# LPD-EPFL/AggregaThor

Measured on NVIDIA H100. Metric: steps/sec (whole box, device-timed, max over ranks) ResNet-50 slim + Krum f=2, higher is better.
Workload: dtype bf16

## Files before the change

### aggregathor_b200/native/op_nn/layers.cu

```cuda

#include <cuda_bf16.h>

#include <agb_device.cuh>

using namespace agb;

namespace {

using bf16 = __nv_bfloat16;

template<typename T> struct Oct;
template<> struct alignas(16) Oct<bf16> { uint4 raw; };
template<> struct alignas(16) Oct<float> { float4 lo, hi; };

__device__ __forceinline__ void unpack8(uint4 const& raw, float (&v)[8]) {
    __nv_bfloat162 const* h = reinterpret_cast<__nv_bfloat162 const*>(&raw);
#pragma unroll
    for (int i = 0; i < 4; ++i) {
        float2 f = __bfloat1622float2(h[i]);
        v[2 * i] = f.x;
        v[2 * i + 1] = f.y;
    }
}
__device__ __forceinline__ uint4 pack8(float const (&v)[8]) {
    uint4 raw;
    __nv_bfloat162* h = reinterpret_cast<__nv_bfloat162*>(&raw);
#pragma unroll
    for (int i = 0; i < 4; ++i)
        h[i] = __floats2bfloat162_rn(v[2 * i], v[2 * i + 1]);
    return raw;
}
__device__ __forceinline__ void unpack8(Oct<bf16> const& o, float (&v)[8]) { unpack8(o.raw, v); }
__device__ __forceinline__ void unpack8(Oct<float> const& o, float (&v)[8]) {
    v[0] = o.lo.x; v[1] = o.lo.y; v[2] = o.lo.z; v[3] = o.lo.w; v[4] = o.hi.x; v[5] = o.hi.y; v[6] = o.hi.z; v[7] = o.hi.w;
}
template<typename T> __device__ __forceinline__ Oct<T> pack_oct(float const (&v)[8]);
template<> __device__ __forceinline__ Oct<bf16> pack_oct<bf16>(float const (&v)[8]) { return Oct<bf16>{pack8(v)}; }
template<> __device__ __forceinline__ Oct<float> pack_oct<float>(float const (&v)[8]) {
    return Oct<float>{make_float4(v[0], v[1], v[2], v[3]), make_float4(v[4], v[5], v[6], v[7])};
}
template<typename T> __device__ __forceinline__ Oct<T> zero_oct() {
    float const z[8] = {0.f, 0.f, 0.f, 0.f, 0.f, 0.f, 0.f, 0.f};
    return pack_oct<T>(z);
}
template<typename T> __device__ __forceinline__ Oct<T> load_oct(T const* p) { return *reinterpret_cast<Oct<T> const*>(p); }
template<typename T> __device__ __forceinline__ void store_oct(T* p, Oct<T> const& o) { *reinterpret_cast<Oct<T>*>(p) = o; }
__device__ __forceinline__ float to_f(bf16 v) { return __bfloat162float(v); }
__device__ __forceinline__ float to_f(float v) { return v; }
template<typename T> __device__ __forceinline__ T from_f(float v);
template<> __device__ __forceinline__ bf16 from_f<bf16>(float v) { return __float2bfloat16(v); }
template<> __device__ __forceinline__ float from_f<float>(float v) { return v; }

constexpr int kThreads = 256;

// ... 786 lines not shown
            for (int kw = 0; kw < KW; ++kw) {
                int const tw = w + pad_l - kw;
                if (tw < 0 || tw % s)
                    continue;
                int const ow = tw / s;
                if (ow >= OW)
                    continue;
                float v[8];
                unpack8(load_oct(dcol + ((static_cast<long long>(n) * OH + oh) * OW + ow) * ldcol + (kh * KW + kw) * C + o * 8), v);
#pragma unroll
                for (int j = 0; j < 8; ++j)
                    acc[j] += v[j];
            }
        }
        store_oct(dx + i * 8, pack_oct<T>(acc));
    }
}

inline int grid_for(long long work, int threads = kThreads, int cap = agb::sm_count() * 8) {
    long long blocks = (work + threads - 1) / threads;
    if (blocks > cap)
        blocks = cap;
    return blocks < 1 ? 1 : static_cast<int>(blocks);
}

struct SumsPlan {
    int rows_per_cta, strip;
    dim3 grid;
};
inline SumsPlan plan_sums(long long rows_per_group, int C, int groups) {
    int const octets = C >> 3;
    SumsPlan plan;
    plan.strip = 8;
    int const row_lanes = kThreads / plan.strip;
    int const strips = (octets + plan.strip - 1) / plan.strip;
    long long target = (agb::sm_count() * 6 + strips * groups - 1) / (strips * groups);
    if (target < 1)
        target = 1;
    long long rows_per_cta = (rows_per_group + target - 1) / target;
    long long const min_rows = static_cast<long long>(row_lanes) * kRowUnroll;
    if (rows_per_cta < min_rows)
        rows_per_cta = min_rows;
    plan.rows_per_cta = static_cast<int>(rows_per_cta);
    plan.grid = dim3(static_cast<unsigned>((rows_per_group + rows_per_cta - 1) / rows_per_cta), strips, groups);
    return plan;
}


constexpr int kFusedThreads = 512;
constexpr int kFusedScratchBytes = kFusedThreads * 16 * 4;
constexpr int kFusedPivotBytes = 12 * 1024;
constexpr int kFusedStashBytes = 180 * 1024;
using FusedSum = double;
constexpr long long kFusedHalfBytes = 16 + 2ll * 8 * 16384;

struct BnFused {
    bf16 const* a;
    bf16 const* b;
    bf16 const* mask;
    bf16* out;
    bf16* out2;
    float const* gamma;
    float const* beta;
    float* moving_mean;
    float* moving_var;
    float* save_mean;
    float* save_rstd;
    float* dgamma;
    float* dbeta;
    long long group_stride;
    unsigned* state;
    unsigned char* ws;
    long long rows_per_group, rows_per_cta;
    int C, groups, ctas_per_group, stash_vecs, relu, replicas;
    float eps, decay;
};

__device__ __forceinline__ unsigned ld_acquire_gpu(unsigned const* addr) {
    unsigned value;
    asm volatile("ld.acquire.gpu.global.u32 %0, [%1];" : "=r"(value) : "l"(addr) : "memory");
    return value;
}

template<bool BWD>
__global__ void __launch_bounds__(kFusedThreads, 1) bn_fused_kernel(BnFused const p) {
    pdl_trigger();
    pdl_wait();
    extern __shared__ __align__(16) unsigned char fused_smem[];
    float* red = reinterpret_cast<float*>(fused_smem);
    float* pivot_s = reinterpret_cast<float*>(fused_smem + kFusedScratchBytes);
    uint4* stash_a = reinterpret_cast<uint4*>(fused_smem + kFusedScratchBytes + kFusedPivotBytes);
    uint4* stash_b = stash_a + p.stash_vecs;
    int const octets = p.C >> 3;
    __shared__ unsigned slot_shared;
    float* chan = red;
    int const group = blockIdx.x / p.ctas_per_group, chunk = blockIdx.x % p.ctas_per_group;
    if (threadIdx.x == 0)
        slot_shared = __ldcg(p.state) & 1u;
    for (int c0 = threadIdx.x; c0 < p.C; c0 += 4 * kFusedThreads) {
        float first[4], second[4];
#pragma unroll
        for (int u = 0; u < 4; ++u) {
            int const c = c0 + u * kFusedThreads;
            first[u] = second[u] = 0.f;
            if (c < p.C) {
                first[u] = BWD ? p.save_mean[group * p.C + c] : (p.moving_mean ? p.moving_mean[c] : 0.f);
                second[u] = BWD ? p.save_rstd[group * p.C + c] : 0.f;
            }
        }
#pragma unroll
        for (int u = 0; u < 4; ++u) {
            int const c = c0 + u * kFusedThreads;
            if (c < p.C) {
                chan[c] = first[u];
                chan[p.C + c] = second[u];
                if (!BWD)
                    pivot_s[c] = first[u];
            }
        }
    }
    __syncthreads();
    unsigned const slot = slot_shared;
    unsigned char* mine = p.ws + slot * kFusedHalfBytes;
    unsigned* bar = reinterpret_cast<unsigned*>(mine);
    FusedSum* sums = reinterpret_cast<FusedSum*>(mine + 16);
    {
        uint4* other = reinterpret_cast<uint4*>(p.ws + (slot ^ 1u) * kFusedHalfBytes);
        for (long long i = static_cast<long long>(blockIdx.x) * kFusedThreads + threadIdx.x; i < kFusedHalfBytes / 16; i += static_cast<long long>(gridDim.x) * kFusedThreads)
            other[i] = make_uint4(0, 0, 0, 0);
    }
    long long const row_begin = static_cast<long long>(chunk) * p.rows_per_cta;
    long long const row_end = min(p.rows_per_group, row_begin + p.rows_per_cta);
    long long const nvec = row_end > row_begin ? (row_end - row_begin) * octets : 0;
    long long const base = (static_cast<long long>(group) * p.rows_per_group + row_begin) * octets;
    uint4 const* ga = reinterpret_cast<uint4 const*>(p.a) + base;
    uint4 const* gb = p.b ? reinterpret_cast<uint4 const*>(p.b) + base : nullptr;
    uint4* gout2 = (BWD && p.out2) ? reinterpret_cast<uint4*>(p.out2) + base : nullptr;
    uint4 const* gm = (BWD && p.mask) ? reinterpret_cast<uint4 const*>(p.mask) + base : nullptr;
    uint4* gout = reinterpret_cast<uint4*>(p.out) + base;
    int const stride = kFusedThreads - kFusedThreads % octets;
    int const lanes = stride / octets;
    bool const active = static_cast<int>(threadIdx.x) < stride;
    int const o = threadIdx.x % octets, lane = threadIdx.x / octets;
    int const cbase = group * p.C + o * 8;
    float s0[8], s1[8], mu[8], rs[8];
#pragma unroll
    for (int j = 0; j < 8; ++j) {
        s0[j] = 0.f;
        s1[j] = 0.f;
        mu[j] = active ? chan[o * 8 + j] : 0.f;
        rs[j] = active ? chan[p.C + o * 8 + j] : 0.f;
    }
    __syncthreads();
    if (active) {
        constexpr int U = BWD ? 4 : 8;
        for (long long i0 = threadIdx.x; i0 < nvec; i0 += static_cast<long long>(stride) * U) {
            uint4 ra[U], rb[U], rm[U];
#pragma unroll
            for (int u = 0; u < U; ++u) {
                long long const i = i0 + static_cast<long long>(u) * stride;
                if (i < nvec) {
                    ra[u] = ga[i];
                    if (BWD)
                        rb[u] = gb[i];
                    if (BWD && gm)
                        rm[u] = gm[i];
                    if (!BWD && gb && (i & 7) == 0)
                        asm volatile("prefetch.global.L2 [%0];" :: "l"(gb + i));
                }
            }
#pragma unroll
            for (int u = 0; u < U; ++u) {
                long long const i = i0 + static_cast<long long>(u) * stride;
                if (i >= nvec)
                    continue;
                float va[8];
                unpack8(ra[u], va);
                if (!BWD) {
#pragma unroll
                    for (int j = 0; j < 8; ++j) {
                        float const d = va[j] - mu[j];
                        s0[j] += d;
                        s1[j] += d * d;
                    }
                    if (i < p.stash_vecs)
                        stash_a[i] = ra[u];
                } else {
                    if (gm) {
                        float vy[8];
                        unpack8(rm[u], vy);
#pragma unroll
                        for (int j = 0; j < 8; ++j)
                            va[j] = vy[j] > 0.f ? va[j] : 0.f;
                        if (gout2)
                            gout2[i] = pack8(va);
                    }
                    float vx[8];
                    unpack8(rb[u], vx);
#pragma unroll
                    for (int j = 0; j < 8; ++j) {
                        s0[j] += va[j];
                        s1[j] += va[j] * (vx[j] - mu[j]) * rs[j];
                    }
                    if (i < p.stash_vecs) {
                        stash_a[i] = gm ? pack8(va) : ra[u];
                        stash_b[i] = rb[u];
                    }
                }
            }
        }
#pragma unroll
        for (int j = 0; j < 8; ++j) {
            red[lane * (octets * 16) + o * 16 + j] = s0[j];
            red[lane * (octets * 16) + o * 16 + 8 + j] = s1[j];
        }
    }
    __syncthreads();
    if (nvec > 0) {
        for (int t = threadIdx.x; t < octets * 16; t += kFusedThreads) {
            float total = 0.f;
            for (int l = 0; l < lanes; ++l)
                total += red[l * (octets * 16) + t];
            long long const slot_index = (static_cast<long long>(chunk % p.replicas) * p.groups + group) * p.C + (t >> 4) * 8 + (t & 7);
            atomicAdd(sums + slot_index * 2 + ((t >> 3) & 1), static_cast<FusedSum>(total));
        }
    }
    __threadfence();
    __syncthreads();
    if (threadIdx.x == 0) {
        atomicAdd(bar, 1u);
        unsigned spins = 0;
        while (ld_acquire_gpu(bar) < gridDim.x) {
            __nanosleep(200);
            if (++spins > (1u << 22)) {
                printf("[agb] bn_fused_kernel: grid barrier timeout (block %d, %u of %u arrived)\n", static_cast<int>(blockIdx.x), ld_acquire_gpu(bar), gridDim.x);
                __trap();
            }
        }
    }
    __syncthreads();
    if (blockIdx.x == 0 && threadIdx.x == 0)
        *p.state = slot ^ 1u;
    {
        double const n = static_cast<double>(p.rows_per_group), inv_n = 1.0 / n;
        for (int c = threadIdx.x; c < p.C; c += kFusedThreads) {
            long long const idx = static_cast<long long>(group) * p.C + c;
            double2 part[8];
#pragma unroll
            for (int r = 0; r < 8; ++r) {
                part[r] = make_double2(0., 0.);
                if (r < p.replicas)
                    part[r] = __ldcg(reinterpret_cast<double2 const*>(sums + (static_cast<long long>(r) * p.groups * p.C + idx) * 2));
            }
            float const gmc = p.gamma ? p.gamma[c] : 1.f;
            float const aux0 = BWD ? p.save_rstd[idx] : p.beta[c], aux1 = BWD ? p.save_mean[idx] : 0.f;
            double t0 = 0., t1 = 0.;
#pragma unroll
            for (int r = 0; r < 8; ++r) {
                t0 += part[r].x;
                t1 += part[r].y;
            }
            if (!BWD) {
                float const pivot = pivot_s[c];
                double const shifted = t0 * inv_n;
                double const mean = shifted + static_cast<double>(pivot);
                double var = fma(-shifted, shifted, t1 * inv_n);
                if (var < 0.)
                    var = 0.;
                float const rstd = rsqrtf(static_cast<float>(var) + p.eps);
                chan[c] = gmc * rstd;
                chan[p.C + c] = aux0 - static_cast<float>(mean) * gmc * rstd;
                if (chunk == 0) {
                    p.save_mean[idx] = static_cast<float>(mean);
                    p.save_rstd[idx] = rstd;
                    if (p.moving_mean && group == 0) {
                        double const unbiased = n > 1. ? var * n / (n - 1.) : var;
                        p.moving_mean[c] = p.decay * pivot + (1.f - p.decay) * static_cast<float>(mean);
                        p.moving_var[c] = p.decay * p.moving_var[c] + (1.f - p.decay) * static_cast<float>(unbiased);
                    }
                }
            } else {
                float const inv = static_cast<float>(inv_n), rsc = aux0, muc = aux1;
                float const b1 = -gmc * rsc * rsc * static_cast<float>(t1) * inv;
                chan[c] = gmc * rsc;
                chan[p.C + c] = b1;
                chan[2 * p.C + c] = -gmc * rsc * static_cast<float>(t0) * inv - b1 * muc;
                if (chunk == 0) {
                    if (p.dgamma)
                        p.dgamma[group * p.group_stride + c] = static_cast<float>(t1);
                    p.dbeta[group * p.group_stride + c] = static_cast<float>(t0);
                }
            }
        }
    }
    __syncthreads();
    if (!active)
        return;
    float c0[8], c1[8], c2[8];
#pragma unroll
    for (int j = 0; j < 8; ++j) {
        c0[j] = chan[o * 8 + j];
        c1[j] = chan[p.C + o * 8 + j];
        c2[j] = BWD ? chan[2 * p.C + o * 8 + j] : 0.f;
    }
    auto finish = [&](float (&va)[8], float const (&vx)[8]) {
        if (!BWD) {
#pragma unroll
            for (int j = 0; j < 8; ++j) {
                va[j] = va[j] * c0[j] + c1[j] + vx[j];
                if (p.relu)
                    va[j] = fmaxf(va[j], 0.f);
            }
        } else {
#pragma unroll
            for (int j = 0; j < 8; ++j)
                va[j] = c0[j] * va[j] + c1[j] * vx[j] + c2[j];
        }
        return pack8(va);
    };
    long long const resident_end = nvec < p.stash_vecs ? nvec : static_cast<long long>(p.stash_vecs);
    long long i = threadIdx.x;
    if (!BWD && gb) {
        constexpr int R = 4;
        for (; i < resident_end; i += static_cast<long long>(stride) * R) {
            uint4 rb[R];
#pragma unroll
            for (int u = 0; u < R; ++u) {
                long long const k = i + static_cast<long long>(u) * stride;
                if (k < resident_end)
                    rb[u] = gb[k];
            }
#pragma unroll
            for (int u = 0; u < R; ++u) {
                long long const k = i + static_cast<long long>(u) * stride;
                if (k >= resident_end)
                    continue;
                float va[8], vx[8];
                unpack8(stash_a[k], va);
                unpack8(rb[u], vx);
                gout[k] = finish(va, vx);
            }
        }
        i = static_cast<long long>(threadIdx.x) >= resident_end ? threadIdx.x : threadIdx.x + ((resident_end - 1 - threadIdx.x) / stride + 1) * stride;
    } else {
        for (; i < resident_end; i += stride) {
            float va[8], vx[8] = {0.f, 0.f, 0.f, 0.f, 0.f, 0.f, 0.f, 0.f};
            unpack8(stash_a[i], va);
            if (BWD)
                unpack8(stash_b[i], vx);
            gout[i] = finish(va, vx);
        }
    }
    constexpr int V = BWD ? 2 : 4;
    for (; i < nvec; i += static_cast<long long>(stride) * V) {
        uint4 ra[V], rb[V], rm[V];
#pragma unroll
        for (int u = 0; u < V; ++u) {
            long long const k = i + static_cast<long long>(u) * stride;
            if (k < nvec) {
                ra[u] = ga[k];
                if (gb)
                    rb[u] = gb[k];
                if (BWD && gm)
                    rm[u] = gm[k];
            }
        }
#pragma unroll
        for (int u = 0; u < V; ++u) {
            long long const k = i + static_cast<long long>(u) * stride;
            if (k >= nvec)
                continue;
            float va[8], vx[8] = {0.f, 0.f, 0.f, 0.f, 0.f, 0.f, 0.f, 0.f};
            unpack8(ra[u], va);
            if (gb)
                unpack8(rb[u], vx);
            if (BWD && gm) {
                float vy[8];
                unpack8(rm[u], vy);
#pragma unroll
                for (int j = 0; j < 8; ++j)
                    va[j] = vy[j] > 0.f ? va[j] : 0.f;
            }
            gout[k] = finish(va, vx);
        }
    }
}

long long g_fused_max_mb[2] = {72, 40};
long long g_fused_min_rows = 4096;

template<bool BWD>
int launch_bn_fused(BnFused p, long long rows, cudaStream_t s) {
    int const octets = p.C >> 3;
    if ((p.C & 7) || 3 * p.C * 4 > kFusedScratchBytes || p.C * 4 > kFusedPivotBytes || p.groups < 1 || p.groups > agb::sm_count() || rows % p.groups || static_cast<long long>(p.C) * p.groups > 16384)
        return 399;
    static bool configured = false;
    int const smem = kFusedScratchBytes + kFusedPivotBytes + kFusedStashBytes;
    if (!configured) {
        AGB_CUDA_OK(cudaFuncSetAttribute(bn_fused_kernel<BWD>, cudaFuncAttributeMaxDynamicSharedMemorySize, smem));
        configured = true;
    }
    bool const extra = BWD ? p.out2 != nullptr : p.b != nullptr;
    long long const bytes = rows * p.C * 2;
    if (rows < (extra ? g_fused_min_rows / 4 : g_fused_min_rows) || bytes > g_fused_max_mb[BWD ? 1 : 0] << 20)
        return 399;
    p.rows_per_group = rows / p.groups;
    long long const vecs = p.rows_per_group * octets;
    long long const min_vecs = octets * 32ll > 2048 ? octets * 32ll : 2048;
    long long want = (vecs + min_vecs - 1) / min_vecs;
    int const cap = agb::sm_count() / p.groups;
    p.ctas_per_group = static_cast<int>(want < 1 ? 1 : (want > cap ? cap : want));
    p.rows_per_cta = (p.rows_per_group + p.ctas_per_group - 1) / p.ctas_per_group;
    p.stash_vecs = kFusedStashBytes / 16 / (BWD ? 2 : 1);
    long long const room = 16384 / (static_cast<long long>(p.C) * p.groups);
    p.replicas = static_cast<int>(room < 1 ? 1 : (room > 8 ? 8 : room));
    if (p.replicas > p.ctas_per_group)
        p.replicas = p.ctas_per_group;
    AGB_CUDA_OK(launch_pdl(bn_fused_kernel<BWD>, dim3(p.groups * p.ctas_per_group), dim3(kFusedThreads), static_cast<size_t>(smem), s, p));
    AGB_CUDA_OK(cudaGetLastError());
    return 0;
}

template<int MODE, typename T>
int launch_sums(SumsPlan const& plan, cudaStream_t s, T const* a, T const* b, T const* y, float const* mean, float const* rstd, double* out,
                 long long rows_per_group, int C, SumsFinalize const& fin) {
    if (plan.strip == 32)
        AGB_CUDA_OK(launch_pdl(channel_sums_kernel<T, MODE, 32>, dim3(plan.grid), dim3(kThreads), 0, s, a, b, y, mean, rstd, out, rows_per_group, C, plan.rows_per_cta, fin));
    else if (plan.strip == 16)
        AGB_CUDA_OK(launch_pdl(channel_sums_kernel<T, MODE, 16>, dim3(plan.grid), dim3(kThreads), 0, s, a, b, y, mean, rstd, out, rows_per_group, C, plan.rows_per_cta, fin));
    else
        AGB_CUDA_OK(launch_pdl(channel_sums_kernel<T, MODE, 8>, dim3(plan.grid), dim3(kThreads), 0, s, a, b, y, mean, rstd, out, rows_per_group, C, plan.rows_per_cta, fin));
    return 0;
}

template<typename T>
int bn_forward_impl(void const* x, void const* residual, void* y, void const* gamma, void const* beta, void* moving_mean, void* moving_var, void* save_mean, void* save_rstd,
                   void* sums, void* scale, void* shift, long long rows, int C, int groups, float eps, float decay, int relu, void* stream) {
    if ((C & 7) || groups < 1 || rows % groups)
        return 301;
    cudaStream_t s = static_cast<cudaStream_t>(stream);
    long long const rpg = rows / groups;
    SumsFinalize fin{};
    fin.ticket = reinterpret_cast<unsigned*>(static_cast<double*>(sums) + 2 * C * groups);
    fin.gamma = static_cast<float const*>(gamma); fin.beta = static_cast<float const*>(beta);
    fin.save_mean = static_cast<float*>(save_mean); fin.save_rstd = static_cast<float*>(save_rstd);
    fin.scale = static_cast<float*>(scale); fin.shift = static_cast<float*>(shift);
    fin.moving_mean = static_cast<float*>(moving_mean); fin.moving_var = static_cast<float*>(moving_var);
    fin.groups = groups; fin.eps = eps; fin.decay = decay;
    SumsPlan plan = plan_sums(rpg, C, groups);
    if (int status = launch_sums<0, T>(plan, s, static_cast<T const*>(x), nullptr, nullptr, nullptr, nullptr, static_cast<double*>(sums), rpg, C, fin))
        return status;
    long long const octets = rows * (C >> 3);
    AGB_CUDA_OK(launch_pdl(bn_apply_kernel<T>, dim3(grid_for(octets)), dim3(kThreads), 0, s, static_cast<T const*>(x), static_cast<T const*>(residual), static_cast<T*>(y), static_cast<float const*>(scale), static_cast<float const*>(shift), octets, C, rpg, relu));
    AGB_CUDA_OK(cudaGetLastError());
    return 0;
}

template<typename T>
int bn_backward_impl(void const* dy, void const* x, void const* y, void const* gamma, void const* save_mean, void const* save_rstd, void* dx, void* dmasked, void* dgamma, void* dbeta,
                    void* sums, void* coef, long long rows, int C, int groups, long long group_stride, void* stream) {
    if ((C & 7) || groups < 1 || rows % groups)
        return 301;
    cudaStream_t s = static_cast<cudaStream_t>(stream);
    long long const rpg = rows / groups;
    SumsFinalize fin{};
    fin.ticket = reinterpret_cast<unsigned*>(static_cast<double*>(sums) + 2 * C * groups);
    fin.gamma = static_cast<float const*>(gamma);
    fin.save_mean = const_cast<float*>(static_cast<float const*>(save_mean)); fin.save_rstd = const_cast<float*>(static_cast<float const*>(save_rstd));
    fin.scale = static_cast<float*>(coef);
    fin.dgamma = static_cast<float*>(dgamma); fin.dbeta = static_cast<float*>(dbeta);
    fin.groups = groups; fin.group_stride = group_stride;
// ... 155 lines not shown
    size_t const stem_smem = static_cast<size_t>(kh) * W * C * sizeof(T);
    if ((C & 7) != 0 && stem_smem <= 40 * 1024 && static_cast<long long>(N) * OH < (1ll << 31)) {
        AGB_CUDA_OK(launch_pdl(im2col_stem_kernel<T>, dim3(static_cast<unsigned>(N * OH)), dim3(kThreads), stem_smem, static_cast<cudaStream_t>(stream), static_cast<T const*>(x), static_cast<T*>(col), H, W, C, OH, OW, kh, kw, s, pad_t, pad_l, ldcol));
        AGB_CUDA_OK(cudaGetLastError());
        return 0;
    }
    long long const work = (C & 7) == 0 ? static_cast<long long>(N) * OH * OW * kh * kw * (C >> 3) : static_cast<long long>(N) * OH * OW * (ldcol >> 3);
    AGB_CUDA_OK(launch_pdl(im2col_kernel<T>, dim3(grid_for(work, kThreads, agb::sm_count() * 16)), dim3(kThreads), 0, static_cast<cudaStream_t>(stream), static_cast<T const*>(x), static_cast<T*>(col), N, H, W, C, OH, OW, kh, kw, s, pad_t, pad_l, ldcol));
    AGB_CUDA_OK(cudaGetLastError());
    return 0;
}

template<typename T>
int col2im_impl(void const* dcol, void* dx, int N, int H, int W, int C, int OH, int OW, int kh, int kw, int s, int pad_t, int pad_l, long long ldcol, void* stream) {
    if ((C & 7) || (ldcol & 7))
        return 301;
    long long const work = static_cast<long long>(N) * H * W * (C >> 3);
    AGB_CUDA_OK(launch_pdl(col2im_kernel<T>, dim3(grid_for(work, kThreads, agb::sm_count() * 16)), dim3(kThreads), 0, static_cast<cudaStream_t>(stream), static_cast<T const*>(dcol), static_cast<T*>(dx), N, H, W, C, OH, OW, kh, kw, s, pad_t, pad_l, ldcol));
    AGB_CUDA_OK(cudaGetLastError());
    return 0;
}

}

extern "C" {

int agb_bn_forward(void const* x, void const* residual, void* y, void const* gamma, void const* beta, void* moving_mean, void* moving_var, void* save_mean, void* save_rstd,
                   void* sums, void* scale, void* shift, long long rows, int C, int groups, float eps, float decay, int relu, void* stream) {
    return bn_forward_impl<bf16>(x, residual, y, gamma, beta, moving_mean, moving_var, save_mean, save_rstd, sums, scale, shift, rows, C, groups, eps, decay, relu, stream);
}
int agb_bn_forward_f32(void const* x, void const* residual, void* y, void const* gamma, void const* beta, void* moving_mean, void* moving_var, void* save_mean, void* save_rstd,
                   void* sums, void* scale, void* shift, long long rows, int C, int groups, float eps, float decay, int relu, void* stream) {
    return bn_forward_impl<float>(x, residual, y, gamma, beta, moving_mean, moving_var, save_mean, save_rstd, sums, scale, shift, rows, C, groups, eps, decay, relu, stream);
}


int agb_bn_backward(void const* dy, void const* x, void const* y, void const* gamma, void const* save_mean, void const* save_rstd, void* dx, void* dmasked, void* dgamma, void* dbeta,
                    void* sums, void* coef, long long rows, int C, int groups, long long group_stride, void* stream) {
    return bn_backward_impl<bf16>(dy, x, y, gamma, save_mean, save_rstd, dx, dmasked, dgamma, dbeta, sums, coef, rows, C, groups, group_stride, stream);
}
int agb_bn_backward_f32(void const* dy, void const* x, void const* y, void const* gamma, void const* save_mean, void const* save_rstd, void* dx, void* dmasked, void* dgamma, void* dbeta,
                    void* sums, void* coef, long long rows, int C, int groups, long long group_stride, void* stream) {
    return bn_backward_impl<float>(dy, x, y, gamma, save_mean, save_rstd, dx, dmasked, dgamma, dbeta, sums, coef, rows, C, groups, group_stride, stream);
}


int agb_bn_fused_set_limits(long long forward_mb, long long backward_mb, long long min_rows) {
    g_fused_max_mb[0] = forward_mb;
    g_fused_max_mb[1] = backward_mb;
    g_fused_min_rows = min_rows;
    return 0;
}

long long agb_bn_fused_workspace_bytes() {
    return 16 + 2 * kFusedHalfBytes;
}

int agb_bn_forward_fused(void const* x, void const* residual, void* y, void const* gamma, void const* beta, void* moving_mean, void* moving_var, void* save_mean, void* save_rstd,
                         void* ws, long long rows, int C, int groups, float eps, float decay, int relu, void* stream) {
    BnFused p{};
    p.a = static_cast<bf16 const*>(x); p.b = static_cast<bf16 const*>(residual); p.out = static_cast<bf16*>(y);
    p.gamma = static_cast<float const*>(gamma); p.beta = static_cast<float const*>(beta);
    p.moving_mean = static_cast<float*>(moving_mean); p.moving_var = static_cast<float*>(moving_var);
    p.save_mean = static_cast<float*>(save_mean); p.save_rstd = static_cast<float*>(save_rstd);
    p.state = static_cast<unsigned*>(ws); p.ws = static_cast<unsigned char*>(ws) + 16;
    p.C = C; p.groups = groups; p.eps = eps; p.decay = decay; p.relu = relu;
    return launch_bn_fused<false>(p, rows, static_cast<cudaStream_t>(stream));
}

int agb_bn_backward_fused(void const* dy, void const* x, void const* y, void const* gamma, void const* save_mean, void const* save_rstd, void* dx, void* dmasked, void* dgamma,
                          void* dbeta, void* ws, long long rows, int C, int groups, long long group_stride, void* stream) {
    BnFused p{};
    p.a = static_cast<bf16 const*>(dy); p.b = static_cast<bf16 const*>(x); p.mask = static_cast<bf16 const*>(y); p.out = static_cast<bf16*>(dx);
    p.out2 = static_cast<bf16*>(dmasked);
    if (p.out2 && !p.mask)
        return 302;
    p.gamma = static_cast<float const*>(gamma);
    p.save_mean = const_cast<float*>(static_cast<float const*>(save_mean)); p.save_rstd = const_cast<float*>(static_cast<float const*>(save_rstd));
    p.dgamma = static_cast<float*>(dgamma); p.dbeta = static_cast<float*>(dbeta); p.group_stride = group_stride;
    p.state = static_cast<unsigned*>(ws); p.ws = static_cast<unsigned char*>(ws) + 16;
    p.C = C; p.groups = groups;
    return launch_bn_fused<true>(p, rows, static_cast<cudaStream_t>(stream));
}

int agb_colsum(void const* dy, void const* y, void* out, void* sums, long long rows, int C, int groups, long long group_stride, void* stream) {
    return colsum_impl<bf16>(dy, y, out, sums, rows, C, groups, group_stride, stream);
}
int agb_colsum_f32(void const* dy, void const* y, void* out, void* sums, long long rows, int C, int groups, long long group_stride, void* stream) {
    return colsum_impl<float>(dy, y, out, sums, rows, C, groups, group_stride, stream);
}


int agb_add_relu(void const* a, void const* b, void* out, long long n, int relu, void* stream) {
    return add_relu_impl<bf16>(a, b, out, n, relu, stream);
}
int agb_add_relu_f32(void const* a, void const* b, void* out, long long n, int relu, void* stream) {
    return add_relu_impl<float>(a, b, out, n, relu, stream);
}


int agb_subsample_forward(void const* x, void* y, int N, int H, int W, int C, int s, void* stream) {
    return subsample_forward_impl<bf16>(x, y, N, H, W, C, s, stream);
}
int agb_subsample_forward_f32(void const* x, void* y, int N, int H, int W, int C, int s, void* stream) {
    return subsample_forward_impl<float>(x, y, N, H, W, C, s, stream);
}
// ... 84 lines not shown
```

### aggregathor_b200/ops/nn_native.py

```python

import ctypes
import os

import torch

from . import counters

_lib_cache = None
_DISABLED = set(filter(None, os.environ.get("AGB_NATIVE_DISABLE", "").split(",")))
SM_COUNT = 132


def _lib():
  global _lib_cache
  if _lib_cache is None:
    from .. import native
    _lib_cache = native.library("op_nn")
  return _lib_cache


def _stream():
  return ctypes.c_void_p(torch.cuda.current_stream().cuda_stream)


# ... 387 lines not shown
    _conv_implicit(2, dy, x, grad_w, n, h, w, oh, ow, cin, cout, k, stride, pads, splits=splits, groups=groups, group_stride=group_stride)
    if has_bias:
      colsum(_as_rows(dy), out=grad_b, groups=groups, group_stride=group_stride)
  dx = None
  if need_dx:
    dx = torch.empty((n, h, w, cin), dtype=x.dtype, device=x.device)
    _conv_implicit(1, dy, weight, dx, n, h, w, oh, ow, cin, cout, k, stride, pads)
    dx = dx.permute(0, 3, 1, 2)
  fork.join()
  return dx



_workspaces = {}


def _workspace(device, name, numel, dtype):
  key = (device, name, dtype)
  buf = _workspaces.get(key)
  if buf is None or buf.numel() < numel:
    buf = _workspaces[key] = torch.zeros(max(numel, 4096), dtype=dtype, device=device)
  return buf


def _cl_ok(*tensors, dtypes=_DTYPES):
  present = [t for t in tensors if t is not None]
  if not present or present[0].dtype not in dtypes or any(t.dtype != present[0].dtype for t in present):
    return False
  return all(t.dim() != 4 or t.is_contiguous(memory_format=torch.channels_last) for t in present)


def colsum(dy2d, y2d=None, out=None, groups=1, group_stride=0):
  rows, c = dy2d.shape
  if out is None:
    out = torch.empty(c, dtype=torch.float32, device=dy2d.device)
  if c % 8 or dy2d.stride(0) != c:
    src = dy2d.float() if y2d is None else dy2d.float() * (y2d > 0)
    _all_groups(out, groups, group_stride).copy_(src.reshape(groups, rows // groups, c).sum(dim=1) if groups > 1 else src.sum(dim=0))
    return out
  sums = _workspace(dy2d.device, "colsum", 2 * c * groups + 1, torch.float64)
  _check(_fn("agb_colsum", dy2d)(_ptr(dy2d), _ptr(y2d), _ptr(out), _ptr(sums), ctypes.c_longlong(rows), ctypes.c_int(c), ctypes.c_int(groups), ctypes.c_longlong(group_stride), _stream()), "colsum")
  return out


_BN_FUSED = os.environ.get("AGB_BN_FUSED", "1") not in ("", "0")
_BN_UNSUPPORTED = 399


def set_bn_fused(flag):
  global _BN_FUSED
  _BN_FUSED = bool(flag)


def set_bn_fused_limits(forward_mb=72, backward_mb=40, min_rows=4096):
  _lib().agb_bn_fused_set_limits(ctypes.c_longlong(forward_mb), ctypes.c_longlong(backward_mb), ctypes.c_longlong(min_rows))


def _bn_fused_workspace(device, name):
  lib = _lib()
  lib.agb_bn_fused_workspace_bytes.restype = ctypes.c_longlong
  return _workspace(device, name, int(lib.agb_bn_fused_workspace_bytes()), torch.uint8)


def batchnorm_forward(x, gamma, beta, moving_mean, moving_var, decay, eps, relu, groups=1, residual=None):
  if not enabled("bn") or not _cl_ok(x, residual) or x.shape[1] % 8:
    return None
  n, c, h, w = x.shape
  rows = n * h * w
  if residual is not None and (residual.shape != x.shape or not residual.is_contiguous(memory_format=torch.channels_last)):
    return None
  y = torch.empty_like(x, memory_format=torch.channels_last)
  stats = torch.empty((4, groups * c), dtype=torch.float32, device=x.device)
  if _BN_FUSED and x.dtype == torch.bfloat16:
    status = _lib().agb_bn_forward_fused(_ptr(x), _ptr(residual), _ptr(y), _ptr(gamma), _ptr(beta), _ptr(moving_mean), _ptr(moving_var), _ptr(stats[0]), _ptr(stats[1]),
                                         _ptr(_bn_fused_workspace(x.device, "bn_fused_fwd")), ctypes.c_longlong(rows), ctypes.c_int(c), ctypes.c_int(groups),
                                         ctypes.c_float(eps), ctypes.c_float(decay), ctypes.c_int(1 if relu else 0), _stream())
    if status != _BN_UNSUPPORTED:
      _check(status, "bn_forward_fused")
      return y, stats[0], stats[1]
  sums = _workspace(x.device, "bn_sums", 2 * groups * c + 1, torch.float64)
  _check(_fn("agb_bn_forward", x)(_ptr(x), _ptr(residual), _ptr(y), _ptr(gamma), _ptr(beta), _ptr(moving_mean), _ptr(moving_var), _ptr(stats[0]), _ptr(stats[1]), _ptr(sums),
                               _ptr(stats[2]), _ptr(stats[3]), ctypes.c_longlong(rows), ctypes.c_int(c), ctypes.c_int(groups), ctypes.c_float(eps),
                               ctypes.c_float(decay), ctypes.c_int(1 if relu else 0), _stream()), "bn_forward")
  return y, stats[0], stats[1]


def batchnorm_backward(dy, x, y, gamma, mean, rstd, relu, grad_gamma, grad_beta, groups=1, group_stride=0, want_masked=False):
  if not enabled("bn") or not _cl_ok(x, dy, y) or x.shape[1] % 8 or (want_masked and not relu):
    return None
  if not dy.is_contiguous(memory_format=torch.channels_last):
    dy = dy.contiguous(memory_format=torch.channels_last)
  n, c, h, w = x.shape
  rows = n * h * w
  dx = torch.empty_like(x, memory_format=torch.channels_last)
  masked = torch.empty_like(dy, memory_format=torch.channels_last) if want_masked else None
  if _BN_FUSED and x.dtype == torch.bfloat16:
    status = _lib().agb_bn_backward_fused(_ptr(dy), _ptr(x), _ptr(y if relu else None), _ptr(gamma), _ptr(mean), _ptr(rstd), _ptr(dx), _ptr(masked), _ptr(grad_gamma),
                                          _ptr(grad_beta), _ptr(_bn_fused_workspace(x.device, "bn_fused_bwd")), ctypes.c_longlong(rows), ctypes.c_int(c), ctypes.c_int(groups),
                                          ctypes.c_longlong(group_stride), _stream())
    if status != _BN_UNSUPPORTED:
      _check(status, "bn_backward_fused")
      return (dx, masked) if want_masked else dx
  sums = _workspace(x.device, "bn_sums", 2 * groups * c + 1, torch.float64)
  coef = _workspace(x.device, "bn_coef", 3 * groups * c, torch.float32)
  _check(_fn("agb_bn_backward", x)(_ptr(dy), _ptr(x), _ptr(y if relu else None), _ptr(gamma), _ptr(mean), _ptr(rstd), _ptr(dx), _ptr(masked), _ptr(grad_gamma), _ptr(grad_beta),
                                _ptr(sums), _ptr(coef), ctypes.c_longlong(rows), ctypes.c_int(c), ctypes.c_int(groups), ctypes.c_longlong(group_stride), _stream()), "bn_backward")
  return (dx, masked) if want_masked else dx

# ... 217 lines not shown
```

Baseline: 18.59.

## Process BN groups in waves inside fused kernel to lift group-count limits

The fused batchnorm kernel now loops over groups in waves, so a grid sized for a subset of groups handles all groups. Each wave runs its own grid barrier. The workspace grows, and only the slots used by the previous launch get zeroed instead of the whole half-buffer. Launch heuristics change too: CTAs per group are sized by stash capacity, and the size limits now apply per group, so more BN calls (many replicas/groups) stay on the fused path. The cost is extra barriers per wave and new default thresholds that may route some calls differently.

```diff
diff --git a/aggregathor_b200/native/op_nn/layers.cu b/aggregathor_b200/native/op_nn/layers.cu
--- a/aggregathor_b200/native/op_nn/layers.cu
+++ b/aggregathor_b200/native/op_nn/layers.cu
@@ -1,5 +1,8 @@
 
 #include <cuda_bf16.h>
+
+#include <cstdlib>
+#include <cstring>
 
 #include <agb_device.cuh>
 
@@ -892,7 +895,8 @@
 constexpr int kFusedPivotBytes = 12 * 1024;
 constexpr int kFusedStashBytes = 180 * 1024;
 using FusedSum = double;
-constexpr long long kFusedHalfBytes = 16 + 2ll * 8 * 16384;
+constexpr long long kFusedSlots = 1ll << 17;
+constexpr long long kFusedHalfBytes = 16 + 2ll * 8 * kFusedSlots;
 
 struct BnFused {
     bf16 const* a;
@@ -912,7 +916,8 @@
     unsigned* state;
     unsigned char* ws;
     long long rows_per_group, rows_per_cta;
-    int C, groups, ctas_per_group, stash_vecs, relu, replicas;
+    int C, groups, ctas_per_group, groups_per_wave, stash_vecs, relu, replicas;
+    unsigned used_vecs;
     float eps, decay;
 };
 
@@ -932,32 +937,17 @@
     uint4* stash_a = reinterpret_cast<uint4*>(fused_smem + kFusedScratchBytes + kFusedPivotBytes);
     uint4* stash_b = stash_a + p.stash_vecs;
     int const octets = p.C >> 3;
-    __shared__ unsigned slot_shared;
+    __shared__ unsigned slot_shared, other_used_shared;
     float* chan = red;
-    int const group = blockIdx.x / p.ctas_per_group, chunk = blockIdx.x % p.ctas_per_group;
-    if (threadIdx.x == 0)
-        slot_shared = __ldcg(p.state) & 1u;
-    for (int c0 = threadIdx.x; c0 < p.C; c0 += 4 * kFusedThreads) {
-        float first[4], second[4];
-#pragma unroll
-        for (int u = 0; u < 4; ++u) {
-            int const c = c0 + u * kFusedThreads;
-            first[u] = second[u] = 0.f;
-            if (c < p.C) {
-                first[u] = BWD ? p.save_mean[group * p.C + c] : (p.moving_mean ? p.moving_mean[c] : 0.f);
-                second[u] = BWD ? p.save_rstd[group * p.C + c] : 0.f;
-            }
-        }
-#pragma unroll
-        for (int u = 0; u < 4; ++u) {
-            int const c = c0 + u * kFusedThreads;
-            if (c < p.C) {
-                chan[c] = first[u];
-                chan[p.C + c] = second[u];
-                if (!BWD)
-                    pivot_s[c] = first[u];
-            }
-        }
+    int const lane_group = blockIdx.x / p.ctas_per_group, chunk = blockIdx.x % p.ctas_per_group;
+    if (threadIdx.x == 0) {
+        unsigned const s = __ldcg(p.state) & 1u;
+        slot_shared = s;
+        other_used_shared = __ldcg(p.state + 1 + (s ^ 1u));
+    }
+    if (!BWD) {
+        for (int c = threadIdx.x; c < p.C; c += kFusedThreads)
+            pivot_s[c] = p.moving_mean ? p.moving_mean[c] : 0.f;
     }
     __syncthreads();
     unsigned const slot = slot_shared;
@@ -966,273 +956,300 @@
     FusedSum* sums = reinterpret_cast<FusedSum*>(mine + 16);
     {
         uint4* other = reinterpret_cast<uint4*>(p.ws + (slot ^ 1u) * kFusedHalfBytes);
-        for (long long i = static_cast<long long>(blockIdx.x) * kFusedThreads + threadIdx.x; i < kFusedHalfBytes / 16; i += static_cast<long long>(gridDim.x) * kFusedThreads)
+        for (long long i = static_cast<long long>(blockIdx.x) * kFusedThreads + threadIdx.x; i < other_used_shared; i += static_cast<long long>(gridDim.x) * kFusedThreads)
             other[i] = make_uint4(0, 0, 0, 0);
+        if (blockIdx.x == 0 && threadIdx.x == 0)
+            p.state[1 + slot] = p.used_vecs;
     }
     long long const row_begin = static_cast<long long>(chunk) * p.rows_per_cta;
     long long const row_end = min(p.rows_per_group, row_begin + p.rows_per_cta);
     long long const nvec = row_end > row_begin ? (row_end - row_begin) * octets : 0;
-    long long const base = (static_cast<long long>(group) * p.rows_per_group + row_begin) * octets;
-    uint4 const* ga = reinterpret_cast<uint4 const*>(p.a) + base;
-    uint4 const* gb = p.b ? reinterpret_cast<uint4 const*>(p.b) + base : nullptr;
-    uint4* gout2 = (BWD && p.out2) ? reinterpret_cast<uint4*>(p.out2) + base : nullptr;
-    uint4 const* gm = (BWD && p.mask) ? reinterpret_cast<uint4 const*>(p.mask) + base : nullptr;
-    uint4* gout = reinterpret_cast<uint4*>(p.out) + base;
     int const stride = kFusedThreads - kFusedThreads % octets;
     int const lanes = stride / octets;
     bool const active = static_cast<int>(threadIdx.x) < stride;
     int const o = threadIdx.x % octets, lane = threadIdx.x / octets;
-    int const cbase = group * p.C + o * 8;
-    float s0[8], s1[8], mu[8], rs[8];
-#pragma unroll
-    for (int j = 0; j < 8; ++j) {
-        s0[j] = 0.f;
-        s1[j] = 0.f;
-        mu[j] = active ? chan[o * 8 + j] : 0.f;
-        rs[j] = active ? chan[p.C + o * 8 + j] : 0.f;
-    }
-    __syncthreads();
-    if (active) {
-        constexpr int U = BWD ? 4 : 8;
-        for (long long i0 = threadIdx.x; i0 < nvec; i0 += static_cast<long long>(stride) * U) {
-            uint4 ra[U], rb[U], rm[U];
-#pragma unroll
-            for (int u = 0; u < U; ++u) {
-                long long const i = i0 + static_cast<long long>(u) * stride;
-                if (i < nvec) {
-                    ra[u] = ga[i];
-                    if (BWD)
-                        rb[u] = gb[i];
-                    if (BWD && gm)
-                        rm[u] = gm[i];
-                    if (!BWD && gb && (i & 7) == 0)
-                        asm volatile("prefetch.global.L2 [%0];" :: "l"(gb + i));
-                }
-            }
-#pragma unroll
-            for (int u = 0; u < U; ++u) {
-                long long const i = i0 + static_cast<long long>(u) * stride;
-                if (i >= nvec)
-                    continue;
-                float va[8];
-                unpack8(ra[u], va);
-                if (!BWD) {
-#pragma unroll
-                    for (int j = 0; j < 8; ++j) {
-                        float const d = va[j] - mu[j];
-                        s0[j] += d;
-                        s1[j] += d * d;
-                    }
-                    if (i < p.stash_vecs)
-                        stash_a[i] = ra[u];
-                } else {
-                    if (gm) {
-                        float vy[8];
-                        unpack8(rm[u], vy);
-#pragma unroll
-                        for (int j = 0; j < 8; ++j)
-                            va[j] = vy[j] > 0.f ? va[j] : 0.f;
-                        if (gout2)
-                            gout2[i] = pack8(va);
-                    }
-                    float vx[8];
-                    unpack8(rb[u], vx);
-#pragma unroll
-                    for (int j = 0; j < 8; ++j) {
-                        s0[j] += va[j];
-                        s1[j] += va[j] * (vx[j] - mu[j]) * rs[j];
-                    }
-                    if (i < p.stash_vecs) {
-                        stash_a[i] = gm ? pack8(va) : ra[u];
-                        stash_b[i] = rb[u];
+    long long const resident_end = nvec < p.stash_vecs ? nvec : static_cast<long long>(p.stash_vecs);
+    int const waves = (p.groups + p.groups_per_wave - 1) / p.groups_per_wave;
+    for (int wave = 0; wave < waves; ++wave) {
+        int const group = wave * p.groups_per_wave + lane_group;
+        bool const busy = group < p.groups;
+        long long const base = (static_cast<long long>(group) * p.rows_per_group + row_begin) * octets;
+        uint4 const* ga = reinterpret_cast<uint4 const*>(p.a) + base;
+        uint4 const* gb = p.b ? reinterpret_cast<uint4 const*>(p.b) + base : nullptr;
+        uint4* gout2 = (BWD && p.out2) ? reinterpret_cast<uint4*>(p.out2) + base : nullptr;
+        uint4 const* gm = (BWD && p.mask) ? reinterpret_cast<uint4 const*>(p.mask) + base : nullptr;
+        uint4* gout = reinterpret_cast<uint4*>(p.out) + base;
+        FusedSum* gsums = sums + static_cast<long long>(group) * p.replicas * p.C * 2;
+        __syncthreads();
+        if (BWD && busy) {
+            for (int c = threadIdx.x; c < p.C; c += kFusedThreads) {
+                chan[c] = p.save_mean[group * p.C + c];
+                chan[p.C + c] = p.save_rstd[group * p.C + c];
+            }
+            __syncthreads();
+        }
+        float s0[8], s1[8], mu[8], rs[8];
+#pragma unroll
+        for (int j = 0; j < 8; ++j) {
+            s0[j] = 0.f;
+            s1[j] = 0.f;
+            mu[j] = active && busy ? (BWD ? chan[o * 8 + j] : pivot_s[o * 8 + j]) : 0.f;
+            rs[j] = active && busy && BWD ? chan[p.C + o * 8 + j] : 0.f;
+        }
+        __syncthreads();
+        if (active && busy) {
+            constexpr int U = BWD ? 4 : 8;
+            for (long long i0 = threadIdx.x; i0 < nvec; i0 += static_cast<long long>(stride) * U) {
+                uint4 ra[U], rb[U], rm[U];
+#pragma unroll
+                for (int u = 0; u < U; ++u) {
+                    long long const i = i0 + static_cast<long long>(u) * stride;
+                    if (i < nvec) {
+                        ra[u] = ga[i];
+                        if (BWD)
+                            rb[u] = gb[i];
+                        if (BWD && gm)
+                            rm[u] = gm[i];
+                        if (!BWD && gb && (i & 7) == 0)
+                            asm volatile("prefetch.global.L2 [%0];" :: "l"(gb + i));
                     }
                 }
-            }
-        }
-#pragma unroll
-        for (int j = 0; j < 8; ++j) {
-            red[lane * (octets * 16) + o * 16 + j] = s0[j];
-            red[lane * (octets * 16) + o * 16 + 8 + j] = s1[j];
-        }
-    }
-    __syncthreads();
-    if (nvec > 0) {
-        for (int t = threadIdx.x; t < octets * 16; t += kFusedThreads) {
-            float total = 0.f;
-            for (int l = 0; l < lanes; ++l)
-                total += red[l * (octets * 16) + t];
-            long long const slot_index = (static_cast<long long>(chunk % p.replicas) * p.groups + group) * p.C + (t >> 4) * 8 + (t & 7);
-            atomicAdd(sums + slot_index * 2 + ((t >> 3) & 1), static_cast<FusedSum>(total));
-        }
-    }
-    __threadfence();
-    __syncthreads();
-    if (threadIdx.x == 0) {
-        atomicAdd(bar, 1u);
-        unsigned spins = 0;
-        while (ld_acquire_gpu(bar) < gridDim.x) {
-            __nanosleep(200);
-            if (++spins > (1u << 22)) {
-                printf("[agb] bn_fused_kernel: grid barrier timeout (block %d, %u of %u arrived)\n", static_cast<int>(blockIdx.x), ld_acquire_gpu(bar), gridDim.x);
-                __trap();
-            }
-        }
-    }
-    __syncthreads();
-    if (blockIdx.x == 0 && threadIdx.x == 0)
-        *p.state = slot ^ 1u;
-    {
-        double const n = static_cast<double>(p.rows_per_group), inv_n = 1.0 / n;
-        for (int c = threadIdx.x; c < p.C; c += kFusedThreads) {
-            long long const idx = static_cast<long long>(group) * p.C + c;
-            double2 part[8];
-#pragma unroll
-            for (int r = 0; r < 8; ++r) {
-                part[r] = make_double2(0., 0.);
-                if (r < p.replicas)
-                    part[r] = __ldcg(reinterpret_cast<double2 const*>(sums + (static_cast<long long>(r) * p.groups * p.C + idx) * 2));
-            }
-            float const gmc = p.gamma ? p.gamma[c] : 1.f;
-            float const aux0 = BWD ? p.save_rstd[idx] : p.beta[c], aux1 = BWD ? p.save_mean[idx] : 0.f;
-            double t0 = 0., t1 = 0.;
-#pragma unroll
-            for (int r = 0; r < 8; ++r) {
-                t0 += part[r].x;
-                t1 += part[r].y;
-            }
-            if (!BWD) {
-                float const pivot = pivot_s[c];
-                double const shifted = t0 * inv_n;
-                double const mean = shifted + static_cast<double>(pivot);
-                double var = fma(-shifted, shifted, t1 * inv_n);
-                if (var < 0.)
-                    var = 0.;
-                float const rstd = rsqrtf(static_cast<float>(var) + p.eps);
-                chan[c] = gmc * rstd;
-                chan[p.C + c] = aux0 - static_cast<float>(mean) * gmc * rstd;
-                if (chunk == 0) {
-                    p.save_mean[idx] = static_cast<float>(mean);
-                    p.save_rstd[idx] = rstd;
-                    if (p.moving_mean && group == 0) {
-                        double const unbiased = n > 1. ? var * n / (n - 1.) : var;
-                        p.moving_mean[c] = p.decay * pivot + (1.f - p.decay) * static_cast<float>(mean);
-                        p.moving_var[c] = p.decay * p.moving_var[c] + (1.f - p.decay) * static_cast<float>(unbiased);
+#pragma unroll
+                for (int u = 0; u < U; ++u) {
+                    long long const i = i0 + static_cast<long long>(u) * stride;
+                    if (i >= nvec)
+                        continue;
+                    float va[8];
+                    unpack8(ra[u], va);
+                    if (!BWD) {
+#pragma unroll
+                        for (int j = 0; j < 8; ++j) {
+                            float const d = va[j] - mu[j];
+                            s0[j] += d;
+                            s1[j] += d * d;
+                        }
+                        if (i < p.stash_vecs)
+                            stash_a[i] = ra[u];
+                    } else {
+                        if (gm) {
+                            float vy[8];
+                            unpack8(rm[u], vy);
+#pragma unroll
+                            for (int j = 0; j < 8; ++j)
+                                va[j] = vy[j] > 0.f ? va[j] : 0.f;
+                            if (gout2)
+                                gout2[i] = pack8(va);
+                        }
+                        float vx[8];
+                        unpack8(rb[u], vx);
+#pragma unroll
+                        for (int j = 0; j < 8; ++j) {
+                            s0[j] += va[j];
+                            s1[j] += va[j] * (vx[j] - mu[j]) * rs[j];
+                        }
+                        if (i < p.stash_vecs) {
+                            stash_a[i] = gm ? pack8(va) : ra[u];
+                            stash_b[i] = rb[u];
+                        }
                     }
                 }
+            }
+#pragma unroll
+            for (int j = 0; j < 8; ++j) {
+                red[lane * (octets * 16) + o * 16 + j] = s0[j];
+                red[lane * (octets * 16) + o * 16 + 8 + j] = s1[j];
+            }
+        }
+        __syncthreads();
+        if (busy && nvec > 0) {
+            for (int t = threadIdx.x; t < octets * 16; t += kFusedThreads) {
+                float total = 0.f;
+                for (int l = 0; l < lanes; ++l)
+                    total += red[l * (octets * 16) + t];
+                long long const slot_index = static_cast<long long>(chunk % p.replicas) * p.C + (t >> 4) * 8 + (t & 7);
+                atomicAdd(gsums + slot_index * 2 + ((t >> 3) & 1), static_cast<FusedSum>(total));
+            }
+        }
+        __threadfence();
+        __syncthreads();
+        if (threadIdx.x == 0) {
+            unsigned const target = static_cast<unsigned>(wave + 1) * gridDim.x;
+            atomicAdd(bar, 1u);
+            unsigned spins = 0;
+            while (ld_acquire_gpu(bar) < target) {
+                __nanosleep(200);
+                if (++spins > (1u << 22)) {
+                    printf("[agb] bn_fused_kernel: grid barrier timeout (block %d, wave %d, %u of %u arrived)\n", static_cast<int>(blockIdx.x), wave, ld_acquire_gpu(bar), target);
+                    __trap();
+                }
+            }
+        }
+        __syncthreads();
+        if (wave == 0 && blockIdx.x == 0 && threadIdx.x == 0)
+            *p.state = slot ^ 1u;
+        if (!busy)
+            continue;
+        {
+            double const n = static_cast<double>(p.rows_per_group), inv_n = 1.0 / n;
+            for (int c = threadIdx.x; c < p.C; c += kFusedThreads) {
+                long long const idx = static_cast<long long>(group) * p.C + c;
+                double2 part[8];
+#pragma unroll
+                for (int r = 0; r < 8; ++r) {
+                    part[r] = make_double2(0., 0.);
+                    if (r < p.replicas)
+                        part[r] = __ldcg(reinterpret_cast<double2 const*>(gsums + (static_cast<long long>(r) * p.C + c) * 2));
+                }
+                float const gmc = p.gamma ? p.gamma[c] : 1.f;
+                float const aux0 = BWD ? p.save_rstd[idx] : p.beta[c], aux1 = BWD ? p.save_mean[idx] : 0.f;
+                double t0 = 0., t1 = 0.;
+#pragma unroll
+                for (int r = 0; r < 8; ++r) {
+                    t0 += part[r].x;
+                    t1 += part[r].y;
+                }
+                if (!BWD) {
+                    float const pivot = pivot_s[c];
+                    double const shifted = t0 * inv_n;
+                    double const mean = shifted + static_cast<double>(pivot);
+                    double var = fma(-shifted, shifted, t1 * inv_n);
+                    if (var < 0.)
+                        var = 0.;
+                    float const rstd = rsqrtf(static_cast<float>(var) + p.eps);
+                    chan[c] = gmc * rstd;
+                    chan[p.C + c] = aux0 - static_cast<float>(mean) * gmc * rstd;
+                    if (chunk == 0) {
+                        p.save_mean[idx] = static_cast<float>(mean);
+                        p.save_rstd[idx] = rstd;
+                        if (p.moving_mean && group == 0) {
+                            double const unbiased = n > 1. ? var * n / (n - 1.) : var;
+                            p.moving_mean[c] = p.decay * pivot + (1.f - p.decay) * static_cast<float>(mean);
+                            p.moving_var[c] = p.decay * p.moving_var[c] + (1.f - p.decay) * static_cast<float>(unbiased);
+                        }
+                    }
+                } else {
+                    float const inv = static_cast<float>(inv_n), rsc = aux0, muc = aux1;
+                    float const b1 = -gmc * rsc * rsc * static_cast<float>(t1) * inv;
+                    chan[c] = gmc * rsc;
+                    chan[p.C + c] = b1;
+                    chan[2 * p.C + c] = -gmc * rsc * static_cast<float>(t0) * inv - b1 * muc;
+                    if (chunk == 0) {
+                        if (p.dgamma)
+                            p.dgamma[group * p.group_stride + c] = static_cast<float>(t1);
+                        p.dbeta[group * p.group_stride + c] = static_cast<float>(t0);
+                    }
+                }
+            }
+        }
+        __syncthreads();
+        if (!active)
+            continue;
+        float c0[8], c1[8], c2[8];
+#pragma unroll
+        for (int j = 0; j < 8; ++j) {
+            c0[j] = chan[o * 8 + j];
+            c1[j] = chan[p.C + o * 8 + j];
+            c2[j] = BWD ? chan[2 * p.C + o * 8 + j] : 0.f;
+        }
+        auto finish = [&](float (&va)[8], float const (&vx)[8]) {
+            if (!BWD) {
+#pragma unroll
+                for (int j = 0; j < 8; ++j) {
+                    va[j] = va[j] * c0[j] + c1[j] + vx[j];
+                    if (p.relu)
+                        va[j] = fmaxf(va[j], 0.f);
+                }
             } else {
-                float const inv = static_cast<float>(inv_n), rsc = aux0, muc = aux1;
-                float const b1 = -gmc * rsc * rsc * static_cast<float>(t1) * inv;
-                chan[c] = gmc * rsc;
-                chan[p.C + c] = b1;
-                chan[2 * p.C + c] = -gmc * rsc * static_cast<float>(t0) * inv - b1 * muc;
-                if (chunk == 0) {
-                    if (p.dgamma)
-                        p.dgamma[group * p.group_stride + c] = static_cast<float>(t1);
-                    p.dbeta[group * p.group_stride + c] = static_cast<float>(t0);
+#pragma unroll
+                for (int j = 0; j < 8; ++j)
+                    va[j] = c0[j] * va[j] + c1[j] * vx[j] + c2[j];
+            }
+            return pack8(va);
+        };
+        long long i = threadIdx.x;
+        if (!BWD && gb) {
+            constexpr int R = 4;
+            for (; i < resident_end; i += static_cast<long long>(stride) * R) {
+                uint4 rb[R];
+#pragma unroll
+                for (int u = 0; u < R; ++u) {
+                    long long const k = i + static_cast<long long>(u) * stride;
+                    if (k < resident_end)
+                        rb[u] = gb[k];
                 }
-            }
-        }
-    }
-    __syncthreads();
-    if (!active)
-        return;
-    float c0[8], c1[8], c2[8];
-#pragma unroll
-    for (int j = 0; j < 8; ++j) {
-        c0[j] = chan[o * 8 + j];
-        c1[j] = chan[p.C + o * 8 + j];
-        c2[j] = BWD ? chan[2 * p.C + o * 8 + j] : 0.f;
-    }
-    auto finish = [&](float (&va)[8], float const (&vx)[8]) {
-        if (!BWD) {
-#pragma unroll
-            for (int j = 0; j < 8; ++j) {
-                va[j] = va[j] * c0[j] + c1[j] + vx[j];
-                if (p.relu)
-                    va[j] = fmaxf(va[j], 0.f);
-            }
+#pragma unroll
+                for (int u = 0; u < R; ++u) {
+                    long long const k = i + static_cast<long long>(u) * stride;
+                    if (k >= resident_end)
+                        continue;
+                    float va[8], vx[8];
+                    unpack8(stash_a[k], va);
+                    unpack8(rb[u], vx);
+                    gout[k] = finish(va, vx);
+                }
+            }
+            i = static_cast<long long>(threadIdx.x) >= resident_end ? threadIdx.x : threadIdx.x + ((resident_end - 1 - threadIdx.x) / stride + 1) * stride;
         } else {
-#pragma unroll
-            for (int j = 0; j < 8; ++j)
-                va[j] = c0[j] * va[j] + c1[j] * vx[j] + c2[j];
-        }
-        return pack8(va);
-    };
-    long long const resident_end = nvec < p.stash_vecs ? nvec : static_cast<long long>(p.stash_vecs);
-    long long i = threadIdx.x;
-    if (!BWD && gb) {
-        constexpr int R = 4;
-        for (; i < resident_end; i += static_cast<long long>(stride) * R) {
-            uint4 rb[R];
-#pragma unroll
-            for (int u = 0; u < R; ++u) {
-                long long const k = i + static_cast<long long>(u) * stride;
-                if (k < resident_end)
-                    rb[u] = gb[k];
-            }
-#pragma unroll
-            for (int u = 0; u < R; ++u) {
-                long long const k = i + static_cast<long long>(u) * stride;
-                if (k >= resident_end)
+            for (; i < resident_end; i += stride) {
+                float va[8], vx[8] = {0.f, 0.f, 0.f, 0.f, 0.f, 0.f, 0.f, 0.f};
+                unpack8(stash_a[i], va);
+                if (BWD)
+                    unpack8(stash_b[i], vx);
+                gout[i] = finish(va, vx);
+            }
+        }
+        constexpr int V = BWD ? 2 : 4;
+        long long const first = i;
+        long long const last = first < nvec ? first + (nvec - 1 - first) / stride * stride : first - 1;
+        for (long long top = last; top >= first; top -= static_cast<long long>(stride) * V) {
+            uint4 ra[V], rb[V], rm[V];
+#pragma unroll
+            for (int u = 0; u < V; ++u) {
+                long long const k = top - static_cast<long long>(u) * stride;
+                if (k >= first) {
+                    ra[u] = ga[k];
+                    if (gb)
+                        rb[u] = gb[k];
+                    if (BWD && gm)
+                        rm[u] = gm[k];
+                }
+            }
+#pragma unroll
+            for (int u = 0; u < V; ++u) {
+                long long const k = top - static_cast<long long>(u) * stride;
+                if (k < first)
                     continue;
-                float va[8], vx[8];
-                unpack8(stash_a[k], va);
-                unpack8(rb[u], vx);
+                float va[8], vx[8] = {0.f, 0.f, 0.f, 0.f, 0.f, 0.f, 0.f, 0.f};
+                unpack8(ra[u], va);
+                if (gb)
+                    unpack8(rb[u], vx);
+                if (BWD && gm) {
+                    float vy[8];
+                    unpack8(rm[u], vy);
+#pragma unroll
+                    for (int j = 0; j < 8; ++j)
+                        va[j] = vy[j] > 0.f ? va[j] : 0.f;
+                }
                 gout[k] = finish(va, vx);
             }
         }
-        i = static_cast<long long>(threadIdx.x) >= resident_end ? threadIdx.x : threadIdx.x + ((resident_end - 1 - threadIdx.x) / stride + 1) * stride;
-    } else {
-        for (; i < resident_end; i += stride) {
-            float va[8], vx[8] = {0.f, 0.f, 0.f, 0.f, 0.f, 0.f, 0.f, 0.f};
-            unpack8(stash_a[i], va);
-            if (BWD)
-                unpack8(stash_b[i], vx);
-            gout[i] = finish(va, vx);
-        }
-    }
-    constexpr int V = BWD ? 2 : 4;
-    for (; i < nvec; i += static_cast<long long>(stride) * V) {
-        uint4 ra[V], rb[V], rm[V];
-#pragma unroll
-        for (int u = 0; u < V; ++u) {
-            long long const k = i + static_cast<long long>(u) * stride;
-            if (k < nvec) {
-                ra[u] = ga[k];
-                if (gb)
-                    rb[u] = gb[k];
-                if (BWD && gm)
-                    rm[u] = gm[k];
-            }
-        }
-#pragma unroll
-        for (int u = 0; u < V; ++u) {
-            long long const k = i + static_cast<long long>(u) * stride;
-            if (k >= nvec)
-                continue;
-            float va[8], vx[8] = {0.f, 0.f, 0.f, 0.f, 0.f, 0.f, 0.f, 0.f};
-            unpack8(ra[u], va);
-            if (gb)
-                unpack8(rb[u], vx);
-            if (BWD && gm) {
-                float vy[8];
-                unpack8(rm[u], vy);
-#pragma unroll
-                for (int j = 0; j < 8; ++j)
-                    va[j] = vy[j] > 0.f ? va[j] : 0.f;
-            }
-            gout[k] = finish(va, vx);
-        }
-    }
-}
-
-long long g_fused_max_mb[2] = {72, 40};
-long long g_fused_min_rows = 4096;
+    }
+}
+
+long long g_fused_max_mb[2] = {-1, -1};
+long long g_fused_min_rows = -1;
+constexpr int kWaveGroupsMax = 8;
+constexpr long long kSmallGroupBytes = 8ll << 20;
+bool g_fused_waves = [] {
+    char const* env = std::getenv("AGB_BN_WAVES");
+    return env == nullptr || (env[0] != '\0' && std::strcmp(env, "0") != 0);
+}();
 
 template<bool BWD>
 int launch_bn_fused(BnFused p, long long rows, cudaStream_t s) {
     int const octets = p.C >> 3;
-    if ((p.C & 7) || 3 * p.C * 4 > kFusedScratchBytes || p.C * 4 > kFusedPivotBytes || p.groups < 1 || p.groups > agb::sm_count() || rows % p.groups || static_cast<long long>(p.C) * p.groups > 16384)
+    int const sms = agb::sm_count();
+    if ((p.C & 7) || 3 * p.C * 4 > kFusedScratchBytes || p.C * 4 > kFusedPivotBytes || p.groups < 1 || rows % p.groups)
         return 399;
     static bool configured = false;
     int const smem = kFusedScratchBytes + kFusedPivotBytes + kFusedStashBytes;
@@ -1240,23 +1257,52 @@
         AGB_CUDA_OK(cudaFuncSetAttribute(bn_fused_kernel<BWD>, cudaFuncAttributeMaxDynamicSharedMemorySize, smem));
         configured = true;
     }
+    p.rows_per_group = rows / p.groups;
+    p.stash_vecs = kFusedStashBytes / 16 / (BWD ? 2 : 1);
+    long long const vecs = p.rows_per_group * octets;
     bool const extra = BWD ? p.out2 != nullptr : p.b != nullptr;
-    long long const bytes = rows * p.C * 2;
-    if (rows < (extra ? g_fused_min_rows / 4 : g_fused_min_rows) || bytes > g_fused_max_mb[BWD ? 1 : 0] << 20)
-        return 399;
-    p.rows_per_group = rows / p.groups;
-    long long const vecs = p.rows_per_group * octets;
-    long long const min_vecs = octets * 32ll > 2048 ? octets * 32ll : 2048;
-    long long want = (vecs + min_vecs - 1) / min_vecs;
-    int const cap = agb::sm_count() / p.groups;
-    p.ctas_per_group = static_cast<int>(want < 1 ? 1 : (want > cap ? cap : want));
-    p.rows_per_cta = (p.rows_per_group + p.ctas_per_group - 1) / p.ctas_per_group;
-    p.stash_vecs = kFusedStashBytes / 16 / (BWD ? 2 : 1);
-    long long const room = 16384 / (static_cast<long long>(p.C) * p.groups);
-    p.replicas = static_cast<int>(room < 1 ? 1 : (room > 8 ? 8 : room));
+    int const d = BWD ? 1 : 0;
+    if (g_fused_waves) {
+        long long const max_mb = g_fused_max_mb[d] >= 0 ? g_fused_max_mb[d] : (BWD ? 32 : (extra ? 8 : 64));
+        long long const min_rows = g_fused_min_rows >= 0 ? g_fused_min_rows : 0;
+        if (p.rows_per_group < (extra ? min_rows / 4 : min_rows) || p.rows_per_group * p.C * 2 > max_mb << 20)
+            return 399;
+        long long const min_vecs = octets * 32ll > 2048 ? octets * 32ll : 2048;
+        long long ctas = sms / kWaveGroupsMax;
+        if (p.rows_per_group * p.C * 2 > kSmallGroupBytes) {
+            long long want = (vecs + p.stash_vecs - 1) / p.stash_vecs;
+            want = want < 1 ? 1 : (want > sms ? sms : want);
+            ctas = sms / (sms / want);
+        }
+        ctas = ctas < 1 ? 1 : ctas;
+        long long const most = (vecs + min_vecs - 1) / min_vecs;
+        p.ctas_per_group = static_cast<int>(ctas < most ? ctas : (most < 1 ? 1 : most));
+        p.groups_per_wave = sms / p.ctas_per_group;
+        if (p.groups_per_wave > p.groups)
+            p.groups_per_wave = p.groups;
+        long long const room = 4096 / p.C;
+        p.replicas = static_cast<int>(room < 1 ? 1 : (room > 8 ? 8 : room));
+    } else {
+        long long const max_mb = g_fused_max_mb[d] >= 0 ? g_fused_max_mb[d] : (BWD ? 40 : 72);
+        long long const min_rows = g_fused_min_rows >= 0 ? g_fused_min_rows : 4096;
+        if (p.groups > sms || static_cast<long long>(p.C) * p.groups > 16384 || rows < (extra ? min_rows / 4 : min_rows) || rows * p.C * 2 > max_mb << 20)
+            return 399;
+        long long const min_vecs = octets * 32ll > 2048 ? octets * 32ll : 2048;
+        long long want = (vecs + min_vecs - 1) / min_vecs;
+        int const cap = sms / p.groups;
+        p.ctas_per_group = static_cast<int>(want < 1 ? 1 : (want > cap ? cap : want));
+        p.groups_per_wave = p.groups;
+        long long const room = 16384 / (static_cast<long long>(p.C) * p.groups);
+        p.replicas = static_cast<int>(room < 1 ? 1 : (room > 8 ? 8 : room));
+    }
     if (p.replicas > p.ctas_per_group)
         p.replicas = p.ctas_per_group;
-    AGB_CUDA_OK(launch_pdl(bn_fused_kernel<BWD>, dim3(p.groups * p.ctas_per_group), dim3(kFusedThreads), static_cast<size_t>(smem), s, p));
+    long long const slots = static_cast<long long>(p.groups) * p.replicas * p.C;
+    if (slots > kFusedSlots)
+        return 399;
+    p.used_vecs = static_cast<unsigned>(1 + slots);
+    p.rows_per_cta = (p.rows_per_group + p.ctas_per_group - 1) / p.ctas_per_group;
+    AGB_CUDA_OK(launch_pdl(bn_fused_kernel<BWD>, dim3(p.groups_per_wave * p.ctas_per_group), dim3(kFusedThreads), static_cast<size_t>(smem), s, p));
     AGB_CUDA_OK(cudaGetLastError());
     return 0;
 }
@@ -1518,6 +1564,11 @@
     return 0;
 }
 
+int agb_bn_fused_set_waves(int waves) {
+    g_fused_waves = waves != 0;
+    return 0;
+}
+
 long long agb_bn_fused_workspace_bytes() {
     return 16 + 2 * kFusedHalfBytes;
 }
diff --git a/aggregathor_b200/ops/nn_native.py b/aggregathor_b200/ops/nn_native.py
--- a/aggregathor_b200/ops/nn_native.py
+++ b/aggregathor_b200/ops/nn_native.py
@@ -463,8 +463,12 @@
   _BN_FUSED = bool(flag)
 
 
-def set_bn_fused_limits(forward_mb=72, backward_mb=40, min_rows=4096):
+def set_bn_fused_limits(forward_mb=-1, backward_mb=-1, min_rows=-1):
   _lib().agb_bn_fused_set_limits(ctypes.c_longlong(forward_mb), ctypes.c_longlong(backward_mb), ctypes.c_longlong(min_rows))
+
+
+def set_bn_waves(flag):
+  _lib().agb_bn_fused_set_waves(ctypes.c_int(1 if flag else 0))
 
 
 def _bn_fused_workspace(device, name):
```

Result: faster. 19.12 (median of 6 runs) (+2.8%).
